# locuslab/icnn

Measured on AMD Instinct MI355X. Metric: inner-solves/sec (batch x iters), n=159 K=10, higher is better.
Workload: dtype f32 PICNN / f64 dual solve

## Files before the change

### icnn_amd/csrc/be_dual_dev.h

```cpp
#pragma once
#include <hip/hip_runtime.h>
#include <math.h>
#include <type_traits>

#include "be_common.h"
#include "be_kernels.h"
#include "icnn_be.h"

namespace icnn_be {

namespace {

constexpr double BOUND_EPS = 1e-12;
constexpr double ARMIJO_ALPHA = 1e-5;
constexpr double GRAD_TOL = 1e-10;
constexpr double TINY = 1e-10;
constexpr double CYCLE_TOL = 1e-13;
constexpr double NOISE_TOL = 1e-10;
constexpr int NOISE_T0 = 12;
constexpr int ACCEL_T0 = 24;
constexpr int ACCEL_GAP = 6;
constexpr double ACCEL_NEG_RESID = 1e-10;
constexpr double ACCEL_D2MAX = 1e-3;
constexpr double ACCEL_RMAX = 0.98;

template <typename T> struct Cut;
__device__ __noinline__ float numpy_expf(float x) {
#pragma clang fp contract(off)
    if (x != x) return x;
    if (x >= 88.72283935546875f) return __builtin_inff();
    if (x <= -103.97208404541015625f) return 0.0f;
    float q = x * 1.44269504088896341f;
    q = q + 12582912.0f;
    q = q - 12582912.0f;
    float r = __builtin_fmaf(q, -6.93145752e-1f, x);
    r = __builtin_fmaf(q, -1.42860677e-6f, r);
    float num = __builtin_fmaf(5.082762527590693718096e-04f, r, 6.757896990527504603057e-03f);
    num = __builtin_fmaf(num, r, 5.114512081637298353406e-02f);
    num = __builtin_fmaf(num, r, 2.473615434895520810817e-01f);
    num = __builtin_fmaf(num, r, 7.257664613233124478488e-01f);
    num = __builtin_fmaf(num, r, 9.999999999980870924916e-01f);
    float den = __builtin_fmaf(2.159509375685829852307e-02f, r, -2.742335390411667452936e-01f);
    den = __builtin_fmaf(den, r, 1.0f);
    const float poly = num / den;
    return ldexpf(poly, (int)q);
}

template <> struct Cut<float> {
    static constexpr double eps = 1.1920928955078125e-07;
    static __device__ __forceinline__ float sigmoid_neg(float g) {
#pragma clang fp contract(off)
        const float e = numpy_expf(g);
        const float d = 1.0f + e;
        return 1.0f / d;
    }
};
template <> struct Cut<double> {
    static constexpr double eps = 2.220446049250313e-16;
    static __device__ __forceinline__ double sigmoid_neg(double g) { return 1.0 / (1.0 + exp(g)); }
};

__device__ __forceinline__ double softplus_stable(double v) {
    return v > 1.0 ? log1p(exp(-v)) + v : log1p(exp(v));
}

struct Carve {
    int As, zs, ws, sp, yv, dv, Hm, Hp, ints, total;
};
constexpr int IPM_KMAX_WAVES = 20;
__host__ __device__ inline Carve carve(int KT, int rows, int ldA, int n_pad, int cut_bytes, int n_leaves,
                                       bool rl, int nw = 1, bool own_const_rows = true, bool ipm = false,
                                       bool glb = false) {
    Carve c;
    int o = 0;
    auto take = [&](int bytes) { int at = o; o += (bytes + 15) & ~15; return at; };
    c.As = take(glb ? 0 : (rows + (own_const_rows ? 2 : 0)) * ldA * cut_bytes);
    c.zs = take(n_pad * 8);
    c.ws = take(n_pad * 8);
    c.sp = (rl || ipm) ? take(n_pad * 8) : c.ws;
    c.yv = ipm ? take(n_pad * 8) : c.zs;
    c.dv = ipm ? take(n_pad * 8) : c.zs;
    const int hp = (rows + 1) | 1;
    int hm = rows * hp * 8;
    const int scratch = (KT * n_leaves + 2 * KT) * 8;
    if (scratch > hm) hm = scratch;
    c.Hm = take(hm);
    c.Hp = nw > 1 ? take(nw * rows * hp * 8) : c.Hm;
    c.ints = take(KT * 4);
    c.total = o;
    return c;
}

__device__ __forceinline__ double bcast(double x, int src_lane) {
    const int lo = __builtin_amdgcn_readlane(__double2loint(x), src_lane);
    const int hi = __builtin_amdgcn_readlane(__double2hiint(x), src_lane);
    return __hiloint2double(hi, lo);
}

typedef const __attribute__((address_space(3))) double lds_cdouble;
__device__ __forceinline__ void pin(double &v) { asm volatile("" : "+v"(v)); }
__device__ __forceinline__ void pin(float &v) { asm volatile("" : "+v"(v)); }
__device__ __forceinline__ int uni(int v) { return __builtin_amdgcn_readfirstlane(v); }
__device__ __forceinline__ unsigned long long uni(unsigned long long v) {
    const unsigned lo = __builtin_amdgcn_readfirstlane((int)(unsigned)v);
    const unsigned hi = __builtin_amdgcn_readfirstlane((int)(unsigned)(v >> 32));
    return ((unsigned long long)hi << 32) | lo;
}
__device__ __forceinline__ double uni(double v) {
    return __hiloint2double(__builtin_amdgcn_readfirstlane(__double2hiint(v)),
                            __builtin_amdgcn_readfirstlane(__double2loint(v)));
}

struct NoLap { __device__ void operator()(int) const {} };
template <typename CutT, bool HESS, typename LapF = NoLap>
__device__ void contract_mfma_8x8(const CutT *As, int ldA, int k, const CutT *crow, int cbeg, int cend,
                                  const double *ws, const double *zs, double *Hm, int HP, LapF lapf = LapF()) {
    const int lane = thread_id() & 63, kq = lane >> 4, blk = (lane >> 2) & 3, r = lane & 3;
    const int ra = 4 * (blk >> 1) + r, cb = 4 * (blk & 1) + r;
    const bool zcol = HESS && cb == k;
    const CutT *pa = (ra < k ? As + ra * ldA : crow) + kq;
    const CutT *pb = (cb < k ? As + cb * ldA : (zcol ? crow + ldA : crow)) + kq;
    const double *pwz = (zcol ? zs : ws) + kq;
    double acc0 = 0.0, acc1 = 0.0;
    cbeg = uni(cbeg); cend = uni(cend);
    CutT xa[4], xb[4], ya[4], yb[4];
    double xw[4], yw[4];
    auto gather = [&](int c0, CutT (&ga)[4], CutT (&gb)[4], double (&gw)[4]) {
#pragma unroll
        for (int s = 0; s < 4; ++s) {
            ga[s] = pa[c0 + 4 * s];
            gb[s] = pb[c0 + 4 * s];
            if (HESS) gw[s] = pwz[c0 + 4 * s];
        }
    };
    auto stage = [&](int cnext, CutT (&ca)[4], CutT (&cb_)[4], double (&cw)[4], CutT (&na)[4], CutT (&nb)[4],
                     double (&nw)[4]) {
        gather(cnext, na, nb, nw);
        __builtin_amdgcn_sched_barrier(0);
#pragma unroll
        for (int s = 0; s < 4; ++s) {
            const double av = (double)ca[s];
            const double bv = HESS ? (double)cb_[s] * cw[s] : (double)cb_[s];
            if (s & 1) acc1 = __builtin_amdgcn_mfma_f64_4x4x4f64(av, bv, acc1, 0, 0, 0);
            else acc0 = __builtin_amdgcn_mfma_f64_4x4x4f64(av, bv, acc0, 0, 0, 0);
        }
        __builtin_amdgcn_sched_barrier(0);
#pragma unroll
        for (int s = 0; s < 4; ++s) { pin(na[s]); pin(nb[s]); if (HESS) pin(nw[s]); }
    };
    if (cbeg < cend) gather(cbeg, xa, xb, xw);
    __builtin_amdgcn_s_waitcnt(0xc07f);
    lapf(10);
    const int clast = cend - 16;
    for (int c0 = cbeg; c0 < cend; c0 += 32) {
        stage(c0 + 16 < cend ? c0 + 16 : clast, xa, xb, xw, ya, yb, yw);
        if (c0 + 16 < cend) stage(c0 + 32 < cend ? c0 + 32 : clast, ya, yb, yw, xa, xb, xw);
    }
    lapf(11);
    const int row = 4 * (blk >> 1) + kq, col = 4 * (blk & 1) + r;
    const int ncolsB = HESS ? k + 1 : k;
    if (row < k && col < ncolsB) Hm[row * HP + col] = acc0 + acc1;
}

template <typename CutT, bool HESS>
__device__ void contract_mfma_cover2(const CutT *As, int ldA, int k, const CutT *crow, int cbeg, int cend, const double *ws,
                                     const double *zs, double *Hm, int HP) {
    const int lane = thread_id() & 63, r16 = lane & 15, q = lane >> 4;
    cbeg = uni(cbeg); cend = uni(cend);
    constexpr int ZC = 64, NONE = 65;
#pragma unroll 1
    for (int t = 0; t < 2; ++t) {
        const int ra = t == 0 ? r16 : 4 + r16;
        int cb;
        if (t == 0) cb = HESS ? (r16 < 15 ? r16 : ZC) : r16;
        else if (r16 < 4) cb = 16 + r16;
        else if (HESS) cb = r16 == 4 ? ZC : (r16 < 9 ? r16 - 5 : (r16 == 9 ? 15 : NONE));
        else cb = r16 < 8 ? r16 - 4 : NONE;
        const bool zcol = cb == ZC;
        const CutT *pa = (ra < k ? As + ra * ldA : crow) + q;
        const CutT *pb = (cb < k ? As + cb * ldA : (zcol ? crow + ldA : crow)) + q;
        const double *pwz = (zcol ? zs : ws) + q;
        d4 acc = {0.0, 0.0, 0.0, 0.0}, acc_odd = {0.0, 0.0, 0.0, 0.0};
        CutT xa[4], xb[4], ya[4], yb[4];
        double xw[4], yw[4];
        auto gather = [&](int c0, CutT (&ga)[4], CutT (&gb)[4], double (&gw)[4]) {
#pragma unroll
            for (int s = 0; s < 4; ++s) {
                ga[s] = pa[c0 + 4 * s];
                gb[s] = pb[c0 + 4 * s];
                if (HESS) gw[s] = pwz[c0 + 4 * s];
            }
        };
        auto stage = [&](int cnext, CutT (&ca)[4], CutT (&cb_)[4], double (&cw)[4], CutT (&na)[4], CutT (&nb)[4], double (&nw)[4]) {
            gather(cnext, na, nb, nw);
            __builtin_amdgcn_sched_barrier(0);
            double av[4], bv[4];
#pragma unroll
            for (int s = 0; s < 4; ++s) {
                av[s] = (double)ca[s];
                bv[s] = HESS ? (double)cb_[s] * cw[s] : (double)cb_[s];
            }
            __builtin_amdgcn_sched_barrier(0);
#pragma unroll
            for (int s = 0; s < 4; ++s) {
                if (s & 1) acc_odd = __builtin_amdgcn_mfma_f64_16x16x4f64(av[s], bv[s], acc_odd, 0, 0, 0);
                else acc = __builtin_amdgcn_mfma_f64_16x16x4f64(av[s], bv[s], acc, 0, 0, 0);
            }
            __builtin_amdgcn_sched_barrier(0);
#pragma unroll
            for (int s = 0; s < 4; ++s) { pin(na[s]); pin(nb[s]); if (HESS) pin(nw[s]); }
        };
        if (cbeg < cend) gather(cbeg, xa, xb, xw);
        __builtin_amdgcn_s_waitcnt(0xc07f);
        const int clast = cend - 16;
        for (int c0 = cbeg; c0 < cend; c0 += 32) {
            stage(c0 + 16 < cend ? c0 + 16 : clast, xa, xb, xw, ya, yb, yw);
            if (c0 + 16 < cend) stage(c0 + 32 < cend ? c0 + 32 : clast, ya, yb, yw, xa, xb, xw);
        }
        acc += acc_odd;
#pragma unroll
        for (int r = 0; r < 4; ++r) {
            const int row = (t == 0 ? 0 : 4) + q + 4 * r;
            if (row >= k) continue;
            if (zcol) {
                if (t == 0 || row >= 16) Hm[row * HP + k] = acc[r];
            } else if (t == 0) {
                Hm[row * HP + cb] = acc[r];
                if (HESS && row == 15) Hm[cb * HP + 15] = acc[r];
            } else if (cb < k) {
                if (cb >= 16) {
                    Hm[row * HP + cb] = acc[r];
                    if (row < 16) Hm[cb * HP + row] = acc[r];
                } else if (cb < 4) {
                    if (row >= 16) { Hm[row * HP + cb] = acc[r]; Hm[cb * HP + row] = acc[r]; }
                } else if (row == 15) {
                    Hm[15 * HP + 15] = acc[r];
                }
            }
        }
    }
}

template <typename CutT, int KT, bool HESS, typename LapF = NoLap>
__device__ void contract_mfma(const CutT *As, int ldA, int k, const CutT *crow, int cbeg, int cend, const double *ws,
                              const double *zs, double *Hm, int HP, LapF lapf = LapF()) {
    const int lane = thread_id() & 63, r16 = lane & 15, q = lane >> 4;
    const int ncolsB = HESS ? k + 1 : k;
    if (ncolsB <= 8) {
        contract_mfma_8x8<CutT, HESS>(As, ldA, k, crow, cbeg, cend, ws, zs, Hm, HP, lapf);
        return;
    }
    if (KT > 16 && k >= 17 && k <= 20) {
        contract_mfma_cover2<CutT, HESS>(As, ldA, k, crow, cbeg, cend, ws, zs, Hm, HP);
        return;
    }
    cbeg = uni(cbeg); cend = uni(cend);
    for (int ti = 0; ti * 16 < k; ++ti) {
        for (int tj = ti; tj * 16 < ncolsB; ++tj) {
            d4 acc = {0.0, 0.0, 0.0, 0.0}, acc_odd = {0.0, 0.0, 0.0, 0.0};
            const int ra = ti * 16 + r16, cb = tj * 16 + r16;
            const bool zcol = HESS && cb == k;
            const CutT *pa = (ra < k ? As + ra * ldA : crow) + q;
            const CutT *pb = (cb < k ? As + cb * ldA : (zcol ? crow + ldA : crow)) + q;
            const double *pwz = (zcol ? zs : ws) + q;
            CutT xa[4], xb[4], ya[4], yb[4];
            double xw[4], yw[4];
            auto gather = [&](int c0, CutT (&ga)[4], CutT (&gb)[4], double (&gw)[4]) {
#pragma unroll
                for (int s = 0; s < 4; ++s) {
                    ga[s] = pa[c0 + 4 * s];
                    gb[s] = pb[c0 + 4 * s];
                    if (HESS) gw[s] = pwz[c0 + 4 * s];
                }
            };
            auto stage = [&](int cnext, CutT (&ca)[4], CutT (&cb_)[4], double (&cw)[4], CutT (&na)[4],
                             CutT (&nb)[4], double (&nw)[4]) {
                gather(cnext, na, nb, nw);
                __builtin_amdgcn_sched_barrier(0);
                double av[4], bv[4];
#pragma unroll
                for (int s = 0; s < 4; ++s) {
                    av[s] = (double)ca[s];
                    bv[s] = HESS ? (double)cb_[s] * cw[s] : (double)cb_[s];
                }
                __builtin_amdgcn_sched_barrier(0);
#pragma unroll
                for (int s = 0; s < 4; ++s) {
                    if (KT > 16 && (s & 1)) acc_odd = __builtin_amdgcn_mfma_f64_16x16x4f64(av[s], bv[s], acc_odd, 0, 0, 0);
                    else acc = __builtin_amdgcn_mfma_f64_16x16x4f64(av[s], bv[s], acc, 0, 0, 0);
                }
                __builtin_amdgcn_sched_barrier(0);
#pragma unroll
                for (int s = 0; s < 4; ++s) { pin(na[s]); pin(nb[s]); if (HESS) pin(nw[s]); }
            };
            if (cbeg < cend) gather(cbeg, xa, xb, xw);
            __builtin_amdgcn_s_waitcnt(0xc07f);
            const int clast = cend - 16;
            for (int c0 = cbeg; c0 < cend; c0 += 32) {
                stage(c0 + 16 < cend ? c0 + 16 : clast, xa, xb, xw, ya, yb, yw);
                if (c0 + 16 < cend) stage(c0 + 32 < cend ? c0 + 32 : clast, ya, yb, yw, xa, xb, xw);
            }
            if (KT > 16) acc += acc_odd;
#pragma unroll
            for (int r = 0; r < 4; ++r) {
                const int row = ti * 16 + q + 4 * r, col = tj * 16 + r16;
                if (row < k && col < ncolsB) {
                    Hm[row * HP + col] = acc[r];
                    if (tj != ti && col < k) Hm[col * HP + row] = acc[r];
                }
            }
        }
    }
}


__device__ __forceinline__ double rcp_nr(double d) {
    double r = __builtin_amdgcn_rcp(d);
    double e = __builtin_fma(-d, r, 1.0);
    r = __builtin_fma(r, e, r);
    e = __builtin_fma(-d, r, 1.0);
    return __builtin_fma(r, e, r);
}

__device__ __forceinline__ double fast_exp(double x) {
    x = fmin(fmax(x, -750.0), 750.0);
    const double kf = __builtin_rint(x * 1.4426950408889634);
    double r = __builtin_fma(kf, -6.93147180369123816490e-01, x);
    r = __builtin_fma(kf, -1.90821492927058770002e-10, r);
    double p = 1.6059043836821613e-10;
    p = __builtin_fma(p, r, 2.08767569878681e-09);
    p = __builtin_fma(p, r, 2.505210838544172e-08);
    p = __builtin_fma(p, r, 2.755731922398589e-07);
    p = __builtin_fma(p, r, 2.7557319223985893e-06);
    p = __builtin_fma(p, r, 2.48015873015873e-05);
    p = __builtin_fma(p, r, 1.984126984126984e-04);
    p = __builtin_fma(p, r, 1.388888888888889e-03);
    p = __builtin_fma(p, r, 8.333333333333333e-03);
    p = __builtin_fma(p, r, 4.1666666666666664e-02);
    p = __builtin_fma(p, r, 1.6666666666666666e-01);
    p = __builtin_fma(p, r, 0.5);
    p = __builtin_fma(p, r, 1.0);
    p = __builtin_fma(p, r, 1.0);
    return __builtin_amdgcn_ldexp(p, (int)kf);
}
__device__ __forceinline__ double fast_log(double x) {
    double m = __builtin_amdgcn_frexp_mant(x);
    int e = __builtin_amdgcn_frexp_exp(x);
    const bool low = m < 0.70710678118654752;
    m = low ? m + m : m;
    e = low ? e - 1 : e;
    const double s = (m - 1.0) * rcp_nr(m + 1.0);
    const double s2 = s * s;
    double p = 2.0 / 21.0;
    p = __builtin_fma(p, s2, 2.0 / 19.0);
    p = __builtin_fma(p, s2, 2.0 / 17.0);
    p = __builtin_fma(p, s2, 2.0 / 15.0);
    p = __builtin_fma(p, s2, 2.0 / 13.0);
    p = __builtin_fma(p, s2, 2.0 / 11.0);
    p = __builtin_fma(p, s2, 2.0 / 9.0);
    p = __builtin_fma(p, s2, 2.0 / 7.0);
    p = __builtin_fma(p, s2, 2.0 / 5.0);
    p = __builtin_fma(p, s2, 2.0 / 3.0);
    const double lm = __builtin_fma(s * s2, p, s + s);
    const double ed = (double)e;
    return __builtin_fma(ed, 6.93147180369123816490e-01, __builtin_fma(ed, 1.90821492927058770002e-10, lm));
}

__device__ __forceinline__ double softplus_fast(double v) {
    const bool big = v > 1.0;
    const double u = fast_exp(big ? -v : v);
    const double w = 1.0 + u;
    const double l = __builtin_fma(u - (w - 1.0), __builtin_amdgcn_rcp(w), fast_log(w));
    return big ? l + v : l;
}

__device__ __forceinline__ double sigmoid_fast(double a) { return rcp_nr(1.0 + fast_exp(fmin(-a, 700.0))); }

template <int KT>
__device__ __noinline__ int inertia_not_above_ks(const double *Hm_, int HP, int k, double mu) {
    const int lane = lane_id();
    lds_cdouble *Hm = (lds_cdouble *)Hm_;
// ... 1166 lines not shown
```

### icnn_amd/csrc/be_ipm_dev.h

```cpp
#pragma once

struct Pair {
    double a, b;
    int ok;
};

__device__ __forceinline__ void ipm_swap16(double &x, double &y) {
    const auto lo = __builtin_amdgcn_permlane16_swap((unsigned)__double2loint(x), (unsigned)__double2loint(y), false, false);
    const auto hi = __builtin_amdgcn_permlane16_swap((unsigned)__double2hiint(x), (unsigned)__double2hiint(y), false, false);
    x = __hiloint2double((int)hi[0], (int)lo[0]);
    y = __hiloint2double((int)hi[1], (int)lo[1]);
}
__device__ __forceinline__ void ipm_swap32(double &x, double &y) {
    const auto lo = __builtin_amdgcn_permlane32_swap((unsigned)__double2loint(x), (unsigned)__double2loint(y), false, false);
    const auto hi = __builtin_amdgcn_permlane32_swap((unsigned)__double2hiint(x), (unsigned)__double2hiint(y), false, false);
    x = __hiloint2double((int)hi[0], (int)lo[0]);
    y = __hiloint2double((int)hi[1], (int)lo[1]);
}
template <typename Op>
__device__ __forceinline__ double wave_reduce_dpp(double v, Op op) {
    v = op(v, dpp_move<0xB1>(v));
    v = op(v, dpp_move<0x4E>(v));
    v = op(v, dpp_move<0x141>(v));
    v = op(v, dpp_move<0x140>(v));
// ... 227 lines not shown
                if (ge < T) v[e] = __builtin_fma(ad[hv_wrow(ge)], ad[hv_wcol(ge)] * w[c], v[e]);
                else if (ge < T + K) v[e] = __builtin_fma(ad[ge - T < K ? ge - T : 0], zz[c], v[e]);
                else if (ge < T + 2 * K) v[e] = __builtin_fma(ad[ge - T - K >= 0 && ge - T - K < K ? ge - T - K : 0], yy[c], v[e]);
                else v[e] = __builtin_fma(ry[c], ry[c], v[e]);
            }
        }
        hv_transpose_reduce<N>(v, lane);
        const int idx = hv_index(N, lane);
        if (idx >= 0) Pw[E0 + idx] = v[0];
        ipm_chunks<CutT, K, E0 + EN, EN, NV>(av, w, zz, yy, ry, lane, Pw);
    }
}

template <typename CutT, int K, typename AP>
__device__ __forceinline__ void ipm_load_columns(AP As, int ldA, int k, const int (&jc)[3], CutT (&av)[K][3]) {
#pragma unroll
    for (int c = 0; c < 3; ++c)
#pragma unroll
        for (int i = 0; i < K; ++i) {
            const CutT v = As[(i < k ? i : 0) * ldA + jc[c]];
            av[i][c] = i < k ? v : (CutT)0;
        }
}

template <typename CutT, int K>
__device__ __noinline__ void ipm_pass1_fn(const CutT *As_, int ldA, int k, int n, int n_pad, const double *yv_, double *rys_,
                                          double *Pw_, double z) {
    typedef const __attribute__((address_space(3))) CutT *LdsCut;
    typedef const __attribute__((address_space(3))) double *LdsCDbl;
    typedef __attribute__((address_space(3))) double *LdsDbl;
    LdsCut As = (LdsCut)As_;
    LdsCDbl yv = (LdsCDbl)yv_;
    LdsDbl rys = (LdsDbl)rys_, Pw = (LdsDbl)Pw_;
    ldA = uni(ldA); k = uni(k); n = uni(n); n_pad = uni(n_pad);
    const int lane = lane_id();
    int jc[3];
#pragma unroll
    for (int c = 0; c < 3; ++c) jc[c] = lane + 64 * c < n_pad ? lane + 64 * c : n_pad - 1;
    CutT av[K][3];
    ipm_load_columns<CutT, K>(As, ldA, k, jc, av);
    double y[3];
#pragma unroll
    for (int c = 0; c < 3; ++c) y[c] = yv[jc[c]];
    double zi[K];
#pragma unroll
    for (int i = 0; i < K; ++i) zi[i] = bcast(z, i);
    double w[3], zz[3], yy[3], ry[3];
#pragma unroll
    for (int c = 0; c < 3; ++c) {
        const int j = lane + 64 * c;
        const double grad = fast_log(y[c] * rcp_nr(1.0 - y[c]));
        const double hinv = y[c] * (1.0 - y[c]);
        double gz = 0.0;
#pragma unroll
        for (int i = 0; i < K; ++i) gz += zi[i] * (double)av[i][c];
        const double r = j < n ? grad + gz : 0.0;
        if (j < n_pad) rys[j] = r;
        ry[c] = r;
        w[c] = j < n ? hinv : 0.0;
        zz[c] = j < n ? hinv * r : 0.0;
        yy[c] = j < n ? y[c] : 0.0;
    }
    ipm_chunks<CutT, K, 0, ipm_chunk(K), ipm_nv(K)>(av, w, zz, yy, ry, lane, Pw);
}

template <typename CutT, int K>
__device__ __noinline__ double ipm_pass2_fn(const CutT *As_, int ldA, int k, int n, int n_pad, const double *yv_,
                                            const double *rys_, double *dyv_, double dz) {
    typedef const __attribute__((address_space(3))) CutT *LdsCut;
    typedef const __attribute__((address_space(3))) double *LdsCDbl;
    typedef __attribute__((address_space(3))) double *LdsDbl;
    LdsCut As = (LdsCut)As_;
    LdsCDbl yv = (LdsCDbl)yv_, rys = (LdsCDbl)rys_;
    LdsDbl dyv = (LdsDbl)dyv_;
    ldA = uni(ldA); k = uni(k); n = uni(n); n_pad = uni(n_pad);
    const int lane = lane_id();
    int jc[3];
#pragma unroll
    for (int c = 0; c < 3; ++c) jc[c] = lane + 64 * c < n_pad ? lane + 64 * c : n_pad - 1;
    CutT av[K][3];
    ipm_load_columns<CutT, K>(As, ldA, k, jc, av);
    double y[3], ry[3];
#pragma unroll
    for (int c = 0; c < 3; ++c) { y[c] = yv[jc[c]]; ry[c] = rys[jc[c]]; }
    double di[K];
#pragma unroll
    for (int i = 0; i < K; ++i) di[i] = bcast(dz, i);
    double m = NO_STEP;
#pragma unroll
    for (int c = 0; c < 3; ++c) {
        const int j = lane + 64 * c;
        const double hinv = j < n ? y[c] * (1.0 - y[c]) : 0.0;
        double gd = 0.0;
#pragma unroll
        for (int i = 0; i < K; ++i) gd += di[i] * (double)av[i][c];
        const double dy = -hinv * (ry[c] + gd);
        if (j < n_pad) dyv[j] = dy;
        if (j < n) m = fmin(m, ratio_step_box(y[c], dy));
    }
    return m;
}

struct IpmStep { double m; int neg; };
template <typename CutT, int K>
__device__ __noinline__ IpmStep ipm_pass3_fn(const CutT *As_, int ldA, int k, int n, int n_pad, const double *yv_, double *dyv_,
                                             double dz) {
    typedef const __attribute__((address_space(3))) CutT *LdsCut;
    typedef const __attribute__((address_space(3))) double *LdsCDbl;
    typedef __attribute__((address_space(3))) double *LdsDbl;
    LdsCut As = (LdsCut)As_;
    LdsCDbl yv = (LdsCDbl)yv_;
    LdsDbl dyv = (LdsDbl)dyv_;
    ldA = uni(ldA); k = uni(k); n = uni(n); n_pad = uni(n_pad);
    const int lane = lane_id();
    int jc[3];
#pragma unroll
    for (int c = 0; c < 3; ++c) jc[c] = lane + 64 * c < n_pad ? lane + 64 * c : n_pad - 1;
    CutT av[K][3];
    ipm_load_columns<CutT, K>(As, ldA, k, jc, av);
    double y[3], d0[3];
#pragma unroll
    for (int c = 0; c < 3; ++c) { y[c] = yv[jc[c]]; d0[c] = dyv[jc[c]]; }
    double di[K];
#pragma unroll
    for (int i = 0; i < K; ++i) di[i] = bcast(dz, i);
    double m = NO_STEP;
    int neg = 0;
#pragma unroll
    for (int c = 0; c < 3; ++c) {
        const int j = lane + 64 * c;
        const double hinv = j < n ? y[c] * (1.0 - y[c]) : 0.0;
        double gd = 0.0;
#pragma unroll
        for (int i = 0; i < K; ++i) gd += di[i] * (double)av[i][c];
        const double dy = d0[c] - hinv * gd;
        if (j < n_pad) dyv[j] = dy;
        if (j < n) {
            m = fmin(m, ratio_step_box(y[c], dy));
            neg |= (dy < 0.0 ? 1 : 0) | (dy > 0.0 ? 2 : 0);
        }
    }
    return IpmStep{m, neg};
}

template <typename CutT, int K, bool GSRC = false>
__device__ __noinline__ void ipm_wide1a_fn(const CutT *As_, int ldA, int k, int n, int n_pad, const double *yv_, double *rys_,
                                           double *ws_, double *zs_, double z, int c_first, int c_step) {
    typedef std::conditional_t<GSRC, const __attribute__((address_space(1))) CutT *, const __attribute__((address_space(3))) CutT *> LdsCut;
    typedef const __attribute__((address_space(3))) double *LdsCDbl;
    typedef __attribute__((address_space(3))) double *LdsDbl;
    LdsCut As = (LdsCut)As_;
    LdsCDbl yv = (LdsCDbl)yv_;
    LdsDbl rys = (LdsDbl)rys_, ws = (LdsDbl)ws_, zs = (LdsDbl)zs_;
    ldA = uni(ldA); k = uni(k); n = uni(n); n_pad = uni(n_pad); c_first = uni(c_first); c_step = uni(c_step);
    const int lane = lane_id();
    double zi[K];
#pragma unroll
    for (int i = 0; i < K; ++i) zi[i] = bcast(z, i);
    for (int c0 = c_first; c0 < n_pad; c0 += c_step) {
        int jc[3];
#pragma unroll
        for (int c = 0; c < 3; ++c) jc[c] = c0 + lane + 64 * c < n_pad ? c0 + lane + 64 * c : n_pad - 1;
        CutT av[K][3];
        ipm_load_columns<CutT, K>(As, ldA, k, jc, av);
        double y[3];
#pragma unroll
        for (int c = 0; c < 3; ++c) y[c] = yv[jc[c]];
#pragma unroll
        for (int c = 0; c < 3; ++c) {
            const int j = c0 + lane + 64 * c;
            const double grad = fast_log(y[c] * rcp_nr(1.0 - y[c]));
            const double hinv = y[c] * (1.0 - y[c]);
            double gz = 0.0;
#pragma unroll
            for (int i = 0; i < K; ++i) gz += zi[i] * (double)av[i][c];
            const double r = j < n ? grad + gz : 0.0;
            if (j < n_pad) {
                rys[j] = r;
                ws[j] = j < n ? hinv : 0.0;
                zs[j] = j < n ? hinv * r : 0.0;
            }
        }
    }
}

template <typename CutT, int K, int E0, int EN, int NV, typename AP, typename CP, typename PP>
__device__ __forceinline__ void ipm_wide_sums(AP As, int ldA, int k, int n, int n_pad, CP ws, CP zs, CP yv, CP rys, int lane, PP Pw,
                                              int c_first, int c_step) {
    if constexpr (E0 < NV) {
        constexpr int N = E0 + EN <= NV ? EN : NV - E0, T = K * (K + 1) / 2;
        double v[N];
#pragma unroll
        for (int e = 0; e < N; ++e) v[e] = 0.0;
        for (int c0 = c_first; c0 < n_pad; c0 += c_step) {
            int jc[3];
#pragma unroll
            for (int c = 0; c < 3; ++c) jc[c] = c0 + lane + 64 * c < n_pad ? c0 + lane + 64 * c : n_pad - 1;
            CutT av[K][3];
            ipm_load_columns<CutT, K>(As, ldA, k, jc, av);
            double w[3], zz[3], yy[3], ry[3];
#pragma unroll
            for (int c = 0; c < 3; ++c) {
                const bool in = c0 + lane + 64 * c < n;
                w[c] = ws[jc[c]]; zz[c] = zs[jc[c]]; ry[c] = rys[jc[c]];
                const double yr = yv[jc[c]];
                if (!(c0 + lane + 64 * c < n_pad)) { w[c] = 0.0; zz[c] = 0.0; ry[c] = 0.0; }
                yy[c] = in ? yr : 0.0;
            }
#pragma unroll
            for (int c = 0; c < 3; ++c) {
                double ad[K];
#pragma unroll
                for (int i = 0; i < K; ++i) ad[i] = (double)av[i][c];
#pragma unroll
                for (int e = 0; e < N; ++e) {
                    const int ge = E0 + e;
                    if (ge < T) v[e] = __builtin_fma(ad[hv_wrow(ge)], ad[hv_wcol(ge)] * w[c], v[e]);
                    else if (ge < T + K) v[e] = __builtin_fma(ad[ge - T < K ? ge - T : 0], zz[c], v[e]);
                    else if (ge < T + 2 * K) v[e] = __builtin_fma(ad[ge - T - K >= 0 && ge - T - K < K ? ge - T - K : 0], yy[c], v[e]);
                    else v[e] = __builtin_fma(ry[c], ry[c], v[e]);
                }
            }
        }
        hv_transpose_reduce<N>(v, lane);
        const int idx = hv_index(N, lane);
        if (idx >= 0) Pw[E0 + idx] = v[0];
        ipm_wide_sums<CutT, K, E0 + EN, EN, NV>(As, ldA, k, n, n_pad, ws, zs, yv, rys, lane, Pw, c_first, c_step);
    }
}
template <typename CutT, int K, bool GSRC = false>
__device__ __noinline__ void ipm_wide1b_fn(const CutT *As_, int ldA, int k, int n, int n_pad, const double *ws_, const double *zs_,
                                           const double *yv_, const double *rys_, double *Pw_, int c_first, int c_step) {
    typedef std::conditional_t<GSRC, const __attribute__((address_space(1))) CutT *, const __attribute__((address_space(3))) CutT *> LdsCut;
    typedef const __attribute__((address_space(3))) double *LdsCDbl;
    typedef __attribute__((address_space(3))) double *LdsDbl;
    ldA = uni(ldA); k = uni(k); n = uni(n); n_pad = uni(n_pad); c_first = uni(c_first); c_step = uni(c_step);
    ipm_wide_sums<CutT, K, 0, ipm_chunk(K), ipm_nv(K)>((LdsCut)As_, ldA, k, n, n_pad, (LdsCDbl)ws_, (LdsCDbl)zs_, (LdsCDbl)yv_,
                                                       (LdsCDbl)rys_, lane_id(), (LdsDbl)Pw_, c_first, c_step);
}

template <typename CutT, int K, bool FIRST, bool GSRC = false>
__device__ __noinline__ IpmStep ipm_wide23_fn(const CutT *As_, int ldA, int k, int n, int n_pad, const double *yv_,
                                              const double *rys_, double *dyv_, double dz, int c_first, int c_step) {
    typedef std::conditional_t<GSRC, const __attribute__((address_space(1))) CutT *, const __attribute__((address_space(3))) CutT *> LdsCut;
    typedef const __attribute__((address_space(3))) double *LdsCDbl;
    typedef __attribute__((address_space(3))) double *LdsDbl;
    LdsCut As = (LdsCut)As_;
    LdsCDbl yv = (LdsCDbl)yv_, rys = (LdsCDbl)rys_;
    LdsDbl dyv = (LdsDbl)dyv_;
    ldA = uni(ldA); k = uni(k); n = uni(n); n_pad = uni(n_pad);
    const int lane = lane_id();
    double di[K];
#pragma unroll
    for (int i = 0; i < K; ++i) di[i] = bcast(dz, i);
    double m = NO_STEP;
    int neg = 0;
    c_first = uni(c_first); c_step = uni(c_step);
    for (int c0 = c_first; c0 < n_pad; c0 += c_step) {
        int jc[3];
#pragma unroll
        for (int c = 0; c < 3; ++c) jc[c] = c0 + lane + 64 * c < n_pad ? c0 + lane + 64 * c : n_pad - 1;
        CutT av[K][3];
        ipm_load_columns<CutT, K>(As, ldA, k, jc, av);
        double y[3], b0[3];
#pragma unroll
        for (int c = 0; c < 3; ++c) { y[c] = yv[jc[c]]; b0[c] = FIRST ? rys[jc[c]] : dyv[jc[c]]; }
#pragma unroll
        for (int c = 0; c < 3; ++c) {
            const int j = c0 + lane + 64 * c;
            const double hinv = j < n ? y[c] * (1.0 - y[c]) : 0.0;
            double gd = 0.0;
#pragma unroll
            for (int i = 0; i < K; ++i) gd += di[i] * (double)av[i][c];
            const double dy = FIRST ? -hinv * (b0[c] + gd) : b0[c] - hinv * gd;
            if (j < n_pad) dyv[j] = dy;
            if (j < n) {
                m = fmin(m, ratio_step_box(y[c], dy));
                neg |= (dy < 0.0 ? 1 : 0) | (dy > 0.0 ? 2 : 0);
            }
        }
    }
    return IpmStep{m, neg};
}

#define IPM_K_SWITCH(kk, CALL)                                                                                     \
    switch (hv_padded(kk)) {                                                                                       \
    case 1: case 2: CALL(2); break; case 3: CALL(3); break; case 4: CALL(4); break; case 5: CALL(5); break;        \
    case 6: CALL(6); break; case 7: CALL(7); break; case 8: CALL(8); break; case 10: CALL(10); break;             \
    default: CALL(12); break;                                                                                      \
    }
#define IPM_K_SWITCH_WAVES(kk, CALL)                                                                               \
    switch (hv_padded(kk)) {                                                                                       \
    case 1: case 2: CALL(2); break; case 3: CALL(3); break; case 4: CALL(4); break; case 5: CALL(5); break;        \
    case 6: CALL(6); break; case 7: CALL(7); break; case 8: CALL(8); break; case 10: CALL(10); break;             \
    case 12: CALL(12); break; case 14: CALL(14); break; case 16: CALL(16); break; case 18: CALL(18); break;       \
    default: CALL(20); break;                                                                                      \
    }

struct IpmOut { double z; int status; };
template <typename CutT, int KT, bool GSRC>
__device__ __noinline__ IpmOut ipm_solve_wide_one_fn(const CutT *As, int ldA, int k, int n, int n_pad, double *ws, double *zs, double *rys,
                                                    double *yv, double *dyv, double *Hm, int HP, double h_i);

template <typename CutT, int KT, bool GLB_ROWS = false, typename LapF = NoLap>
__device__ __forceinline__ double ipm_solve(const CutT *As, int ldA, int k, const CutT *crow, int n, int n_pad,
                                            double *ws, double *zs, double *rys, double *yv, double *dyv, double *Hm,
                                            int HP, double h_i, int lane, int *status, LapF lap = LapF()) {
    const bool row = lane < k;
    const bool hv_ok = sizeof(CutT) == 4 && n_pad <= 192 && !GLB_ROWS;
    const bool fast = hv_ok && k >= 2 && k <= IPM_KMAX && ipm_nv(hv_padded(k)) <= n_pad;
    const int KP = hv_padded(k), TP = KP * (KP + 1) / 2;
    if (sizeof(CutT) == 4 && n_pad > 192 && k <= IPM_KMAX_WAVES && ((ipm_nv(k < 2 ? 2 : KP) + 3) & ~3) <= n_pad) {
        if constexpr (sizeof(CutT) == 4) {
            const IpmOut o = ipm_solve_wide_one_fn<CutT, KT, GLB_ROWS>(As, ldA, k, n, n_pad, ws, zs, rys, yv, dyv, Hm, HP, h_i);
            *status = uni(o.status);
            return o.z;
        }
    }
    double z = row ? 1.0 / (double)k : 0.0;
    double s = row ? 1.0 : 0.0;
    double t = 1.0;
    for (int j = lane; j < n_pad; j += 64) yv[j] = 0.5;
    sample_sync<1>();
    *status = 0;
    auto cols_dot = [&](double v, int j) -> double {
        double acc = 0.0;
        for (int i = 0; i < k; ++i) acc += bcast(v, i) * (double)As[i * ldA + j];
        return acc;
    };
    const auto add = [](double x, double y) { return x + y; };
    auto rsum = [&](double v) -> double { return rows_reduce<KT>(row ? v : 0.0, k, add); };
    auto rows_dot = [&](const double *vec) -> double {
        double mine = 0.0;
        for (int i = 0; i < k; ++i) {
            double part = 0.0;
            for (int j = lane; j < n_pad; j += 64) part += (double)As[i * ldA + j] * vec[j];
            part = ipm_sum(part);
            if (lane == i) mine = part;
        }
        return mine;
    };
    double gy = 0.0, near = 1.0;
    for (int it = 0; it < 20; ++it) {
        const bool fresh = fast || it == 0 || near < 1e-4;
        if (fresh && !fast) gy = rows_dot(yv);
        double pri2 = 0.0;
        if (fast) {
#define IPM_P1(KK) ipm_pass1_fn<CutT, KK>(As, ldA, k, n, n_pad, yv, rys, zs, z)
            IPM_K_SWITCH(k, IPM_P1)
#undef IPM_P1
            sample_sync<1>();
            hv_gather<1, true>(zs, 0, Hm, HP, k, lane, 64, hv_entry<true>(lane, k, HP));
            gy = row ? zs[TP + KP + lane] : 0.0;
            pri2 = zs[TP + 2 * KP];
        } else
        for (int j = lane; j < n_pad; j += 64) {
            const double y = yv[j];
            const double grad = fast_log(y * rcp_nr(1.0 - y));
            const double hinv = y * (1.0 - y);
            const double ry = j < n ? grad + cols_dot(z, j) : 0.0;
            rys[j] = ry;
            ws[j] = j < n ? hinv : 0.0;
            zs[j] = j < n ? hinv * ry : 0.0;
            pri2 += ry * ry;
        }
        sample_sync<1>();
        lap(4);
        const double rt = 1.0 - rsum(z);
        double rd = row ? gy + h_i - t + s : 0.0;
        const double pri_res = sqrt((fast ? pri2 : ipm_sum(pri2)) + rt * rt);
        double dual_res = sqrt(rsum(rd * rd));
        lap(8);
        if (pri_res < 1e-8 && dual_res < 1e-8) {
            if (fresh) break;
            gy = rows_dot(yv);
            rd = row ? gy + h_i - t + s : 0.0;
            dual_res = sqrt(rsum(rd * rd));
            if (dual_res < 1e-8) break;
        }
        near = fmax(pri_res, dual_res);
        if (fast) {
        } else if (hv_ok && k >= 2 && k <= HV_K1MAX && hv_pitch(k) <= n_pad) {
            hv_weighted_pass_k<CutT>(As, ldA, k, n, n_pad, ws, zs, zs);
            sample_sync<1>();
            hv_gather<1, true>(zs, hv_pitch(k), Hm, HP, k, lane, 64, hv_entry<true>(lane, k, HP));
        } else {
            contract_mfma<CutT, KT, true>(As, ldA, k, crow, 0, n_pad, ws, zs, Hm, HP);
        }
        sample_sync<1>();
        lap(5);
        const double soz = row ? s * rcp_nr(z) : 1.0;
        const double ghr = row ? Hm[lane * HP + k] : 0.0;
        const double r = rd - ghr - soz * z;
        const int fks = spd_factor_size(k, n_pad);
        const Pair um = fks ? spd_factor2_k(fks, Hm, HP, k, soz, r, 1.0, zs) : spd_solve2_k<KT>(Hm, HP, k, soz, r, 1.0);
        if (!uni(um.ok) || !isfinite(pri_res)) { *status = 1; break; }
        lap(9);
        const double m1 = row ? um.b : 0.0, m1inv = rcp_nr(rsum(m1));
        const double dt_a = (rsum(r * m1) - rt) * m1inv;
        const double dz_a = row ? um.a - dt_a * m1 : 0.0;
        const double ds_a = -soz * (z + dz_a);
        double mall = row ? fmin(ratio_step(z, dz_a), ratio_step(s, ds_a)) : NO_STEP;
        if (fast) {
#define IPM_P2(KK) mall = fmin(mall, ipm_pass2_fn<CutT, KK>(As, ldA, k, n, n_pad, yv, rys, dyv, dz_a))
            IPM_K_SWITCH(k, IPM_P2)
#undef IPM_P2
        } else
        for (int j = lane; j < n_pad; j += 64) {
            const double dy = -ws[j] * (rys[j] + cols_dot(dz_a, j));
            dyv[j] = dy;
            if (j < n) mall = fmin(mall, fmin(ratio_step(yv[j], dy), ratio_step(1.0 - yv[j], -dy)));
        }
        double alpha = fmin(wave_min(mall), 1.0);
        lap(6);
        const double sz = rsum(s * z);
        const double q = rsum((s + alpha * ds_a) * (z + alpha * dz_a)) * rcp_nr(sz);
        const double sig = q * q * q;
        const double mu = sz / (double)k;
        const double rc2 = row ? -(mu * sig - ds_a * dz_a) * rcp_nr(s) : 0.0;
        const double r2 = -(soz * rc2);
        sample_sync<1>();
        const double u2a = fks ? spd_resolve_k(fks, zs, k, r2) : spd_solve2_k<KT>(Hm, HP, k, soz, r2, 0.0).a;
        lap(10);
        const double dt_c = rsum(r2 * m1) * m1inv;
        const double dz_c = row ? u2a - dt_c * m1 : 0.0;
        const double ds_c = -soz * (rc2 + dz_c);
        const double dz = dz_a + dz_c, ds = ds_a + ds_c, dt = dt_a + dt_c;
        mall = row ? fmin(ratio_step(s, ds), ratio_step(z, dz)) : NO_STEP;
        bool neg_y = false, neg_1y = false;
        if (fast) {
            IpmStep st3{NO_STEP, 0};
#define IPM_P3(KK) st3 = ipm_pass3_fn<CutT, KK>(As, ldA, k, n, n_pad, yv, dyv, dz_c)
            IPM_K_SWITCH(k, IPM_P3)
#undef IPM_P3
            mall = fmin(mall, st3.m);
            neg_y = (st3.neg & 1) != 0;
            neg_1y = (st3.neg & 2) != 0;
        } else
        for (int j = lane; j < n_pad; j += 64) {
            const double dy = dyv[j] - ws[j] * cols_dot(dz_c, j);
            dyv[j] = dy;
            if (j < n) {
                mall = fmin(mall, fmin(ratio_step(yv[j], dy), ratio_step(1.0 - yv[j], -dy)));
                neg_y |= dy < 0.0;
                neg_1y |= dy > 0.0;
            }
        }
        const bool some_empty = !__any(row && ds < 0.0) || !__any(row && dz < 0.0) || !__any(neg_y) || !__any(neg_1y);
        const double mwave = wave_min(mall);
        const double gmin = some_empty ? fmin(mwave, 1.0) : mwave;
        alpha = fmax(0.0, fmin(1.0, 0.99 * gmin));
        for (int j = lane; j < n; j += 64) yv[j] += alpha * dyv[j];
        if (!fast) {
            double mdz = 0.0;
            for (int j = 0; j < k; ++j) mdz += Hm[(row ? lane : 0) * HP + j] * bcast(dz, j);
            gy += alpha * (-ghr - mdz);
        }
        t += alpha * dt;
        s += alpha * ds;
        z += alpha * dz;
        sample_sync<1>();
        lap(11);
    }
    return row ? z : 0.0;
}

template <typename CutT, int KT, int NW, bool GSRC = false, typename LapF = NoLap>
__device__ __forceinline__ double ipm_solve_waves(const CutT *As, int ldA, int k, int n, int n_pad, double *ws, double *zs, double *rys,
                                                  double *yv, double *dyv, double *Hq, int HP, double h_i, int tid, int *status,
                                                  LapF lap = LapF()) {
    constexpr int NT = 64 * NW;
    const int lane = tid & 63, wave = uni(tid >> 6);
    const bool row = lane < k;
    const int KP = k < 2 ? 2 : hv_padded(k), TP = KP * (KP + 1) / 2, NVP = (ipm_nv(KP) + 3) & ~3;
    const int c_first = wave * 192, c_step = 192 * NW;
    double *part = dyv;
    double *xch = ws;
    double z = row ? 1.0 / (double)k : 0.0, s = row ? 1.0 : 0.0, t = 1.0;
    for (int j = tid; j < n_pad; j += NT) yv[j] = 0.5;
    sample_sync<NW>();
    *status = 0;
    const auto add = [](double x, double y) { return x + y; };
    auto rsum = [&](double v) -> double { return rows_reduce<KT>(row ? v : 0.0, k, add); };
    for (int it = 0; it < 20; ++it) {
#define IPM_M1A(KK) ipm_wide1a_fn<CutT, KK, GSRC>(As, ldA, k, n, n_pad, yv, rys, ws, zs, z, c_first, c_step)
        IPM_K_SWITCH_WAVES(k, IPM_M1A)
#undef IPM_M1A
        sample_sync<NW>();
#define IPM_M1B(KK) ipm_wide1b_fn<CutT, KK, GSRC>(As, ldA, k, n, n_pad, ws, zs, yv, rys, part + wave * NVP, c_first, c_step)
        IPM_K_SWITCH_WAVES(k, IPM_M1B)
#undef IPM_M1B
        sample_sync<NW>();
        lap(4);
        double gy = 0.0, pri2 = 0.0;
        if (k >= 2) {
            hv_gather<NW, true>(part, NVP, Hq, HP, k, lane, 64, hv_entry<true>(lane, k, HP));
        } else {
            double m = 0.0, g = 0.0;
#pragma unroll
            for (int w = 0; w < NW; ++w) { m += part[w * NVP]; g += part[w * NVP + TP]; }
            if (lane == 0) { Hq[0] = m; Hq[1] = g; }
            sample_sync<1>();
        }
#pragma unroll
        for (int w = 0; w < NW; ++w) {
            gy += row ? part[w * NVP + TP + KP + lane] : 0.0;
            pri2 += part[w * NVP + TP + 2 * KP];
        }
        sample_sync<NW>();
        lap(5);
        const double rt = 1.0 - rsum(z);
        const double rd = row ? gy + h_i - t + s : 0.0;
        const double pri_res = sqrt(pri2 + rt * rt), dual_res = sqrt(rsum(rd * rd));
        lap(8);
        if (pri_res < 1e-8 && dual_res < 1e-8) break;
        const double soz = row ? s * rcp_nr(z) : 1.0;
        const double ghr = row ? Hq[lane * HP + k] : 0.0;
        const double r = rd - ghr - soz * z;
        const int fks = spd_factor_size(k, n_pad);
        const Pair um = fks ? spd_factor2_k(fks, Hq, HP, k, soz, r, 1.0, zs) : spd_solve2_k<KT>(Hq, HP, k, soz, r, 1.0);
        if (!uni(um.ok) || !isfinite(pri_res)) { *status = 1; break; }
        lap(9);
        const double m1 = row ? um.b : 0.0, m1inv = rcp_nr(rsum(m1));
        const double dt_a = (rsum(r * m1) - rt) * m1inv;
        const double dz_a = row ? um.a - dt_a * m1 : 0.0;
        const double ds_a = -soz * (z + dz_a);
        double mall = row ? fmin(ratio_step(z, dz_a), ratio_step(s, ds_a)) : NO_STEP;
#define IPM_M2(KK) mall = fmin(mall, ipm_wide23_fn<CutT, KK, true, GSRC>(As, ldA, k, n, n_pad, yv, rys, dyv, dz_a, c_first, c_step).m)
        IPM_K_SWITCH_WAVES(k, IPM_M2)
#undef IPM_M2
        {
            const double wm = wave_min(mall);
            if (lane == 0) xch[wave] = wm;
            sample_sync<NW>();
            mall = xch[0];
#pragma unroll
            for (int w = 1; w < NW; ++w) mall = fmin(mall, xch[w]);
            sample_sync<NW>();
        }
        double alpha = fmin(mall, 1.0);
        lap(6);
        const double sz = rsum(s * z);
        const double q = rsum((s + alpha * ds_a) * (z + alpha * dz_a)) * rcp_nr(sz);
        const double sig = q * q * q;
        const double mu = sz / (double)k;
        const double rc2 = row ? -(mu * sig - ds_a * dz_a) * rcp_nr(s) : 0.0;
        const double r2 = -(soz * rc2);
        const double u2a = fks ? spd_resolve_k(fks, zs, k, r2) : spd_solve2_k<KT>(Hq, HP, k, soz, r2, 0.0).a;
        lap(10);
        const double dt_c = rsum(r2 * m1) * m1inv;
        const double dz_c = row ? u2a - dt_c * m1 : 0.0;
        const double ds_c = -soz * (rc2 + dz_c);
        const double dz = dz_a + dz_c, ds = ds_a + ds_c, dt = dt_a + dt_c;
        mall = row ? fmin(ratio_step(s, ds), ratio_step(z, dz)) : NO_STEP;
        IpmStep st3{NO_STEP, 0};
#define IPM_M3(KK) st3 = ipm_wide23_fn<CutT, KK, false, GSRC>(As, ldA, k, n, n_pad, yv, rys, dyv, dz_c, c_first, c_step)
        IPM_K_SWITCH_WAVES(k, IPM_M3)
#undef IPM_M3
        mall = fmin(mall, st3.m);
        bool neg_y, neg_1y;
        {
            const double wm = wave_min(mall);
            const int flags = (__any(st3.neg & 1) ? 1 : 0) | (__any(st3.neg & 2) ? 2 : 0);
            if (lane == 0) { xch[wave] = wm; xch[NW + wave] = (double)flags; }
            sample_sync<NW>();
            mall = xch[0];
            int fl = (int)xch[NW];
#pragma unroll
            for (int w = 1; w < NW; ++w) { mall = fmin(mall, xch[w]); fl |= (int)xch[NW + w]; }
            neg_y = (fl & 1) != 0;
            neg_1y = (fl & 2) != 0;
            sample_sync<NW>();
        }
        const bool some_empty = !__any(row && ds < 0.0) || !__any(row && dz < 0.0) || !neg_y || !neg_1y;
        const double gmin = some_empty ? fmin(mall, 1.0) : mall;
        alpha = fmax(0.0, fmin(1.0, 0.99 * gmin));
        for (int j = tid; j < n; j += NT) yv[j] += alpha * dyv[j];
        t += alpha * dt;
        s += alpha * ds;
        z += alpha * dz;
        sample_sync<NW>();
        lap(11);
    }
    return row ? z : 0.0;
}

template <typename CutT, int KT, bool GSRC>
__device__ __noinline__ IpmOut ipm_solve_wide_one_fn(const CutT *As, int ldA, int k, int n, int n_pad, double *ws, double *zs, double *rys,
                                                    double *yv, double *dyv, double *Hm, int HP, double h_i) {
    ldA = uni(ldA); k = uni(k); n = uni(n); n_pad = uni(n_pad); HP = uni(HP);
    int st = 0;
    const double z = ipm_solve_waves<CutT, KT, 1, GSRC>(As, ldA, k, n, n_pad, ws, zs, rys, yv, dyv, Hm, HP, h_i, lane_id(), &st);
    return IpmOut{z, st};
}
```

Measured before the change: 41.45 million.

## Split fast IPM path into noinline function with LDS pointers and parked temporaries

Moves the fast interior-point solve into its own noinline function. Inside it, scratch pointers are cast to the LDS address space and uniform values are forced into scalar registers. Per-row temporaries (dz_a, ds_a, m1, rc2) are spilled to a small parked LDS buffer, carved from the ws slot, instead of being kept live across the k-switch pass calls. The goal is to cut register pressure and generic-address overhead in the inlined hot loop, at the cost of a function call and extra LDS round-trips.

```diff
diff --git a/icnn_amd/csrc/be_dual_dev.h b/icnn_amd/csrc/be_dual_dev.h
--- a/icnn_amd/csrc/be_dual_dev.h
+++ b/icnn_amd/csrc/be_dual_dev.h
@@ -68,6 +68,7 @@
     int As, zs, ws, sp, yv, dv, Hm, Hp, ints, total;
 };
 constexpr int IPM_KMAX_WAVES = 20;
+constexpr int IPM_PARK = 4 * 16;
 __host__ __device__ inline Carve carve(int KT, int rows, int ldA, int n_pad, int cut_bytes, int n_leaves,
                                        bool rl, int nw = 1, bool own_const_rows = true, bool ipm = false,
                                        bool glb = false) {
@@ -76,7 +77,7 @@
     auto take = [&](int bytes) { int at = o; o += (bytes + 15) & ~15; return at; };
     c.As = take(glb ? 0 : (rows + (own_const_rows ? 2 : 0)) * ldA * cut_bytes);
     c.zs = take(n_pad * 8);
-    c.ws = take(n_pad * 8);
+    c.ws = take((ipm && n_pad < IPM_PARK ? IPM_PARK : n_pad) * 8);
     c.sp = (rl || ipm) ? take(n_pad * 8) : c.ws;
     c.yv = ipm ? take(n_pad * 8) : c.zs;
     c.dv = ipm ? take(n_pad * 8) : c.zs;
diff --git a/icnn_amd/csrc/be_ipm_dev.h b/icnn_amd/csrc/be_ipm_dev.h
--- a/icnn_amd/csrc/be_ipm_dev.h
+++ b/icnn_amd/csrc/be_ipm_dev.h
@@ -553,6 +553,121 @@
 __device__ __noinline__ IpmOut ipm_solve_wide_one_fn(const CutT *As, int ldA, int k, int n, int n_pad, double *ws, double *zs, double *rys,
                                                     double *yv, double *dyv, double *Hm, int HP, double h_i);
 
+template <typename CutT, int KT, typename LapF>
+__device__ __noinline__ IpmOut ipm_solve_fast_fn(const CutT *As, int ldA, int k, int n, int n_pad, double *zs_, double *rys_, double *yv_,
+                                                double *dyv_, double *Hm_, int HP, double *park_, double h_i, LapF lap) {
+    typedef __attribute__((address_space(3))) double *LdsDbl;
+    ldA = uni(ldA); k = uni(k); n = uni(n); n_pad = uni(n_pad); HP = uni(HP);
+    const auto lds = [](double *p) { return (LdsDbl)(unsigned long)(unsigned)uni((int)(unsigned)(unsigned long)(LdsDbl)p); };
+    const LdsDbl zs = lds(zs_), rys = lds(rys_), yv = lds(yv_), dyv = lds(dyv_), Hm = lds(Hm_), park = lds(park_);
+    As = (const CutT *)uni((unsigned long long)As);
+    const int lane = lane_id();
+    const bool row = lane < k;
+    const int pl = lane & 15;
+    const int KP = hv_padded(k), TP = KP * (KP + 1) / 2;
+    const int fks = spd_factor_size(k, n_pad);
+    double z = row ? 1.0 / (double)k : 0.0;
+    double s = row ? 1.0 : 0.0;
+    double t = 1.0;
+    for (int j = lane; j < n_pad; j += 64) yv[j] = 0.5;
+    sample_sync<1>();
+    int status = 0;
+    const auto add = [](double x, double y) { return x + y; };
+    auto rsum = [&](double v) -> double { return rows_reduce<KT>(row ? v : 0.0, k, add); };
+    for (int it = 0; it < 20; ++it) {
+#define IPM_P1(KK) ipm_pass1_fn<CutT, KK>(As, ldA, k, n, n_pad, (double *)yv, (double *)rys, (double *)zs, z)
+        IPM_K_SWITCH(k, IPM_P1)
+#undef IPM_P1
+        sample_sync<1>();
+        {
+            HvEntry en = hv_entry<true>(lane, k, HP);
+            for (int e = lane; e < k * (k + 1); e += 64) {
+                if (e != lane) en = hv_entry<true>(e, k, HP);
+                double acc = 0.0;
+                acc += zs[en.idx];
+                Hm[en.dst] = acc;
+            }
+            sample_sync<1>();
+        }
+        const double gy = row ? zs[TP + KP + lane] : 0.0;
+        const double pri2 = zs[TP + 2 * KP];
+        sample_sync<1>();
+        lap(4);
+        const double rt = 1.0 - rsum(z);
+        const double rd = row ? gy + h_i - t + s : 0.0;
+        const double pri_res = sqrt(pri2 + rt * rt);
+        const double dual_res = sqrt(rsum(rd * rd));
+        lap(8);
+        if (pri_res < 1e-8 && dual_res < 1e-8) break;
+        sample_sync<1>();
+        lap(5);
+        double dt_a, m1inv, alpha;
+        {
+            const double soz = row ? s * rcp_nr(z) : 1.0;
+            const double ghr = row ? Hm[lane * HP + k] : 0.0;
+            const double r = rd - ghr - soz * z;
+            const Pair um = fks ? spd_factor2_k(fks, (double *)Hm, HP, k, soz, r, 1.0, (double *)zs) : spd_solve2_k<KT>((double *)Hm, HP, k, soz, r, 1.0);
+            if (!uni(um.ok) || !isfinite(pri_res)) { status = 1; break; }
+            lap(9);
+            const double m1 = row ? um.b : 0.0;
+            m1inv = rcp_nr(rsum(m1));
+            dt_a = (rsum(r * m1) - rt) * m1inv;
+            const double dz_a = row ? um.a - dt_a * m1 : 0.0;
+            const double ds_a = -soz * (z + dz_a);
+            if (lane < 16) { park[lane] = dz_a; park[16 + lane] = ds_a; park[32 + lane] = m1; }
+            double mall = row ? fmin(ratio_step(z, dz_a), ratio_step(s, ds_a)) : NO_STEP;
+#define IPM_P2(KK) mall = fmin(mall, ipm_pass2_fn<CutT, KK>(As, ldA, k, n, n_pad, (double *)yv, (double *)rys, (double *)dyv, dz_a))
+            IPM_K_SWITCH(k, IPM_P2)
+#undef IPM_P2
+            alpha = fmin(wave_min(mall), 1.0);
+        }
+        lap(6);
+        double r2;
+        {
+            const double dz_a = lane < 16 ? park[pl] : 0.0, ds_a = lane < 16 ? park[16 + pl] : -0.0;
+            const double soz = row ? s * rcp_nr(z) : 1.0;
+            const double sz = rsum(s * z);
+            const double q = rsum((s + alpha * ds_a) * (z + alpha * dz_a)) * rcp_nr(sz);
+            const double sig = q * q * q;
+            const double mu = sz / (double)k;
+            const double rc2 = row ? -(mu * sig - ds_a * dz_a) * rcp_nr(s) : 0.0;
+            r2 = -(soz * rc2);
+            if (lane < 16) park[48 + lane] = rc2;
+        }
+        sample_sync<1>();
+        const double u2a = fks ? spd_resolve_k(fks, (double *)zs, k, r2) : spd_solve2_k<KT>((double *)Hm, HP, k, row ? s * rcp_nr(z) : 1.0, r2, 0.0).a;
+        lap(10);
+        double dz, ds, dt, dz_c;
+        {
+            const double m1 = lane < 16 ? park[32 + pl] : 0.0, rc2 = lane < 16 ? park[48 + pl] : 0.0;
+            const double dz_a = lane < 16 ? park[pl] : 0.0, ds_a = lane < 16 ? park[16 + pl] : -0.0;
+            const double soz = row ? s * rcp_nr(z) : 1.0;
+            const double dt_c = rsum(r2 * m1) * m1inv;
+            dz_c = row ? u2a - dt_c * m1 : 0.0;
+            const double ds_c = -soz * (rc2 + dz_c);
+            dz = dz_a + dz_c; ds = ds_a + ds_c; dt = dt_a + dt_c;
+        }
+        double mall = row ? fmin(ratio_step(s, ds), ratio_step(z, dz)) : NO_STEP;
+        IpmStep st3{NO_STEP, 0};
+#define IPM_P3(KK) st3 = ipm_pass3_fn<CutT, KK>(As, ldA, k, n, n_pad, (double *)yv, (double *)dyv, dz_c)
+        IPM_K_SWITCH(k, IPM_P3)
+#undef IPM_P3
+        mall = fmin(mall, st3.m);
+        const bool neg_y = (st3.neg & 1) != 0, neg_1y = (st3.neg & 2) != 0;
+        const bool some_empty = !__any(row && ds < 0.0) || !__any(row && dz < 0.0) || !__any(neg_y) || !__any(neg_1y);
+        const double mwave = wave_min(mall);
+        const double gmin = some_empty ? fmin(mwave, 1.0) : mwave;
+        const double alpha2 = fmax(0.0, fmin(1.0, 0.99 * gmin));
+        for (int j = lane; j < n; j += 64) yv[j] += alpha2 * dyv[j];
+        t += alpha2 * dt;
+        s += alpha2 * ds;
+        z += alpha2 * dz;
+        sample_sync<1>();
+        lap(11);
+    }
+    return IpmOut{row ? z : 0.0, status};
+}
+
 template <typename CutT, int KT, bool GLB_ROWS = false, typename LapF = NoLap>
 __device__ __forceinline__ double ipm_solve(const CutT *As, int ldA, int k, const CutT *crow, int n, int n_pad,
                                             double *ws, double *zs, double *rys, double *yv, double *dyv, double *Hm,
@@ -560,13 +675,22 @@
     const bool row = lane < k;
     const bool hv_ok = sizeof(CutT) == 4 && n_pad <= 192 && !GLB_ROWS;
     const bool fast = hv_ok && k >= 2 && k <= IPM_KMAX && ipm_nv(hv_padded(k)) <= n_pad;
-    const int KP = hv_padded(k), TP = KP * (KP + 1) / 2;
+    const int KP = hv_padded(k);
     if (sizeof(CutT) == 4 && n_pad > 192 && k <= IPM_KMAX_WAVES && ((ipm_nv(k < 2 ? 2 : KP) + 3) & ~3) <= n_pad) {
         if constexpr (sizeof(CutT) == 4) {
             const IpmOut o = ipm_solve_wide_one_fn<CutT, KT, GLB_ROWS>(As, ldA, k, n, n_pad, ws, zs, rys, yv, dyv, Hm, HP, h_i);
             *status = uni(o.status);
             return o.z;
         }
+    }
+    if (fast) {
+        IpmOut o{0.0, 0};
+        if constexpr (sizeof(CutT) == 4 && !GLB_ROWS) {
+            if constexpr (ICNN_BE_PROF) o = ipm_solve_fast_fn<CutT, KT, LapF>(As, ldA, k, n, n_pad, zs, rys, yv, dyv, Hm, HP, ws, h_i, lap);
+            else o = ipm_solve_fast_fn<CutT, KT, NoLap>(As, ldA, k, n, n_pad, zs, rys, yv, dyv, Hm, HP, ws, h_i, NoLap());
+        }
+        *status = uni(o.status);
+        return o.z;
     }
     double z = row ? 1.0 / (double)k : 0.0;
     double s = row ? 1.0 : 0.0;
@@ -593,18 +717,9 @@
     };
     double gy = 0.0, near = 1.0;
     for (int it = 0; it < 20; ++it) {
-        const bool fresh = fast || it == 0 || near < 1e-4;
-        if (fresh && !fast) gy = rows_dot(yv);
+        const bool fresh = it == 0 || near < 1e-4;
+        if (fresh) gy = rows_dot(yv);
         double pri2 = 0.0;
-        if (fast) {
-#define IPM_P1(KK) ipm_pass1_fn<CutT, KK>(As, ldA, k, n, n_pad, yv, rys, zs, z)
-            IPM_K_SWITCH(k, IPM_P1)
-#undef IPM_P1
-            sample_sync<1>();
-            hv_gather<1, true>(zs, 0, Hm, HP, k, lane, 64, hv_entry<true>(lane, k, HP));
-            gy = row ? zs[TP + KP + lane] : 0.0;
-            pri2 = zs[TP + 2 * KP];
-        } else
         for (int j = lane; j < n_pad; j += 64) {
             const double y = yv[j];
             const double grad = fast_log(y * rcp_nr(1.0 - y));
@@ -619,7 +734,7 @@
         lap(4);
         const double rt = 1.0 - rsum(z);
         double rd = row ? gy + h_i - t + s : 0.0;
-        const double pri_res = sqrt((fast ? pri2 : ipm_sum(pri2)) + rt * rt);
+        const double pri_res = sqrt(ipm_sum(pri2) + rt * rt);
         double dual_res = sqrt(rsum(rd * rd));
         lap(8);
         if (pri_res < 1e-8 && dual_res < 1e-8) {
@@ -630,8 +745,7 @@
             if (dual_res < 1e-8) break;
         }
         near = fmax(pri_res, dual_res);
-        if (fast) {
-        } else if (hv_ok && k >= 2 && k <= HV_K1MAX && hv_pitch(k) <= n_pad) {
+        if (hv_ok && k >= 2 && k <= HV_K1MAX && hv_pitch(k) <= n_pad) {
             hv_weighted_pass_k<CutT>(As, ldA, k, n, n_pad, ws, zs, zs);
             sample_sync<1>();
             hv_gather<1, true>(zs, hv_pitch(k), Hm, HP, k, lane, 64, hv_entry<true>(lane, k, HP));
@@ -652,11 +766,6 @@
         const double dz_a = row ? um.a - dt_a * m1 : 0.0;
         const double ds_a = -soz * (z + dz_a);
         double mall = row ? fmin(ratio_step(z, dz_a), ratio_step(s, ds_a)) : NO_STEP;
-        if (fast) {
-#define IPM_P2(KK) mall = fmin(mall, ipm_pass2_fn<CutT, KK>(As, ldA, k, n, n_pad, yv, rys, dyv, dz_a))
-            IPM_K_SWITCH(k, IPM_P2)
-#undef IPM_P2
-        } else
         for (int j = lane; j < n_pad; j += 64) {
             const double dy = -ws[j] * (rys[j] + cols_dot(dz_a, j));
             dyv[j] = dy;
@@ -679,15 +788,6 @@
         const double dz = dz_a + dz_c, ds = ds_a + ds_c, dt = dt_a + dt_c;
         mall = row ? fmin(ratio_step(s, ds), ratio_step(z, dz)) : NO_STEP;
         bool neg_y = false, neg_1y = false;
-        if (fast) {
-            IpmStep st3{NO_STEP, 0};
-#define IPM_P3(KK) st3 = ipm_pass3_fn<CutT, KK>(As, ldA, k, n, n_pad, yv, dyv, dz_c)
-            IPM_K_SWITCH(k, IPM_P3)
-#undef IPM_P3
-            mall = fmin(mall, st3.m);
-            neg_y = (st3.neg & 1) != 0;
-            neg_1y = (st3.neg & 2) != 0;
-        } else
         for (int j = lane; j < n_pad; j += 64) {
             const double dy = dyv[j] - ws[j] * cols_dot(dz_c, j);
             dyv[j] = dy;
@@ -702,7 +802,7 @@
         const double gmin = some_empty ? fmin(mwave, 1.0) : mwave;
         alpha = fmax(0.0, fmin(1.0, 0.99 * gmin));
         for (int j = lane; j < n; j += 64) yv[j] += alpha * dyv[j];
-        if (!fast) {
+        {
             double mdz = 0.0;
             for (int j = 0; j < k; ++j) mdz += Hm[(row ? lane : 0) * HP + j] * bcast(dz, j);
             gy += alpha * (-ghr - mdz);
```

Measured after the change: 41.41 million. No clear change (-0.1%).
